# szaguldo-kamaz/FRI-ReinforcementLearning-C

Measured on AMD Instinct MI355X. Metric: rule-distance evals/sec (rules x envs), higher is better.
Workload: dtype f64; 1 GPU; cfg4_acrobot_64k_x_8k_per_gpu; nant=5, universe_len=41, rules_per_env=65536, envs_per_gpu=8192, exact_hits=4, dist_backend=none, world_size=1

## Files before the change

fri-reinforcementlearning-c_amd/csrc/five_rule_distance.hip:

```cpp
#include <stdlib.h>

#include <type_traits>

#include "device_common.h"

namespace frirl {

__device__ __forceinline__ void item_to_env_chunk(unsigned item, int cpe, int E, bool env_fastest, int &e, int &c)
{
    if (env_fastest) { c = (int)(item / (unsigned)E); e = (int)(item - (unsigned)c * (unsigned)E); }
    else { e = (int)(item / (unsigned)cpe); c = (int)(item - (unsigned)e * (unsigned)cpe); }
}

template <int NANT, bool WRITE, int UNROLL, int NT>
__global__ __launch_bounds__(FRIRL_BLOCK) void rule_distance_kernel(
    const double *__restrict__ u, const double *__restrict__ ve, int U, const double *__restrict__ rb,
    const int32_t *__restrict__ nrules, int maxR, const double *__restrict__ x, double *__restrict__ dists,
    uint32_t *__restrict__ hit, int rules_per_block, int cpe, int E, int env_fastest)
{
    int e, c;
    item_to_env_chunk(blockIdx.x, cpe, E, env_fastest != 0, e, c);
    const int R = nrules[e];
    const int r0 = c * rules_per_block;
    if (r0 >= R) return;
// ... 33 lines not shown
            if (rr < r_end) {
                double d0 = q[0] - v[j][0].x, d1 = q[0] - v[j][0].y;
                double a0 = d0 * d0, a1 = d1 * d1;
#pragma unroll
                for (int k = 1; k < NANT; k++) {
                    d0 = q[k] - v[j][k].x;
                    d1 = q[k] - v[j][k].y;
                    const double s0 = d0 * d0, s1 = d1 * d1;
                    a0 = a0 + s0;
                    a1 = a1 + s1;
                }
                double2 d;
                d.x = __dsqrt_rn(a0);
                d.y = __dsqrt_rn(a1);
                if (WRITE) {
                    if (NT == 1 || NT == 3) { __builtin_nontemporal_store(d.x, out + rr); __builtin_nontemporal_store(d.y, out + rr + 1); }
                    else *reinterpret_cast<double2 *>(out + rr) = d;
                }
                if (d.y == 0.0 && rr + 1 < R) best = min(best, (unsigned)(rr + 1));
                if (d.x == 0.0) best = min(best, (unsigned)rr);
            }
        }
    }
    best = block_min_u32(best, red_s);
    if (threadIdx.x == 0 && best != FRIRL_HIP_NO_HIT) atomicMin(&hit[e], best);
}

template <int NANT>
__device__ __forceinline__ double2 idx_pair_distance(const uint32_t (&w)[NANT], const double (&q)[NANT], const double *__restrict__ tab_s, int U)
{
    double2 t = lds_table_pair(tab_s, w[0]);
    double d0 = q[0] - t.x, d1 = q[0] - t.y;
    double a0 = d0 * d0, a1 = d1 * d1;
#pragma unroll
    for (int k = 1; k < NANT; k++) {
        t = lds_table_pair(tab_s + k * U, w[k]);
        d0 = q[k] - t.x;
        d1 = q[k] - t.y;
        const double s0 = d0 * d0, s1 = d1 * d1;
        a0 = a0 + s0;
        a1 = a1 + s1;
    }
    double2 d;
    d.x = __dsqrt_rn(a0);
    d.y = __dsqrt_rn(a1);
    return d;
}

template <int NANT, bool WRITE, int UNROLL, int BLOCK = FRIRL_BLOCK>
__global__ __launch_bounds__(BLOCK) void rule_distance_idx_kernel(
    const double *__restrict__ u, const double *__restrict__ ve, int U, const uint16_t *__restrict__ uidx,
    const int32_t *__restrict__ nrules, int maxR, const double *__restrict__ x, double *__restrict__ dists,
    uint32_t *__restrict__ hit, int rules_per_block, int cpe, int E, int env_fastest)
{
    extern __shared__ double tab_s[];
    int e, c;
    item_to_env_chunk(blockIdx.x, cpe, E, env_fastest != 0, e, c);
    const int R = nrules[e];
    const int r0 = c * rules_per_block;
    if (r0 >= R) return;
    int r_end = r0 + rules_per_block;
    if (r_end > R) r_end = R;

    __shared__ double q_s[NANT];
    __shared__ unsigned red_s[BLOCK / FRIRL_WAVE];
    for (int i = threadIdx.x; i < NANT * U; i += BLOCK) tab_s[i] = ve[i];
    if (threadIdx.x < NANT) q_s[threadIdx.x] = observe_ve(u, ve, U, threadIdx.x, x[(size_t)e * NANT + threadIdx.x]);
    __syncthreads();
    double q[NANT];
#pragma unroll
    for (int k = 0; k < NANT; k++) q[k] = q_s[k];

    const uint16_t *__restrict__ base = uidx + (size_t)e * NANT * maxR;
    double *__restrict__ out = WRITE ? dists + (size_t)e * maxR : nullptr;
    unsigned best = FRIRL_HIP_NO_HIT;
    constexpr int STEP = BLOCK * 2;

    for (int r = r0 + 2 * (int)threadIdx.x; r < r_end; r += STEP * UNROLL) {
        uint32_t w[UNROLL][NANT];
#pragma unroll
        for (int j = 0; j < UNROLL; j++) {
            const int rr = r + j * STEP;
            if (rr < r_end) {
#pragma unroll
                for (int k = 0; k < NANT; k++) w[j][k] = __builtin_nontemporal_load(reinterpret_cast<const uint32_t *>(base + (size_t)k * maxR + rr));
            }
        }
#pragma unroll
        for (int j = 0; j < UNROLL; j++) {
            const int rr = r + j * STEP;
            if (rr < r_end) {
                const double2 d = idx_pair_distance<NANT>(w[j], q, tab_s, U);
                if (WRITE) { __builtin_nontemporal_store(d.x, out + rr); __builtin_nontemporal_store(d.y, out + rr + 1); }
                if (d.y == 0.0 && rr + 1 < R) best = min(best, (unsigned)(rr + 1));
                if (d.x == 0.0) best = min(best, (unsigned)rr);
            }
        }
    }
    best = wave_min_u32(best);
    if ((threadIdx.x & (FRIRL_WAVE - 1)) == 0) red_s[threadIdx.x / FRIRL_WAVE] = best;
    __syncthreads();
    if (threadIdx.x == 0) {
        unsigned m = red_s[0];
        for (int w = 1; w < BLOCK / FRIRL_WAVE; w++) m = red_s[w] < m ? red_s[w] : m;
        if (m != FRIRL_HIP_NO_HIT) atomicMin(&hit[e], m);
    }
}

typedef uint32_t u32x2_t __attribute__((ext_vector_type(2)));
static constexpr int RD_XCDS = 8;

template <int BITS>
__device__ __forceinline__ double pk_table_entry(const double *__restrict__ tab_k, uint32_t w, int sh)
{
    constexpr uint32_t FM = ((1u << BITS) - 1u) << 3;
    const uint32_t off = (sh >= 3 ? (w >> (sh - 3)) : (w << (3 - sh))) & FM;
    return *reinterpret_cast<const double *>(reinterpret_cast<const char *>(tab_k) + off);
}

template <int NANT, int BITS>
__device__ __forceinline__ double2 pk_pair_distance(const u32x2_t (&w)[Packed<BITS>::words(NANT)], const double (&q)[NANT],
                                                    const double *__restrict__ tab_s)
{
    constexpr int FPW = Packed<BITS>::FPW, TS = 1 << BITS;
    double d0 = q[0] - pk_table_entry<BITS>(tab_s, w[0].x, 0), d1 = q[0] - pk_table_entry<BITS>(tab_s, w[0].y, 0);
    double a0 = d0 * d0, a1 = d1 * d1;
#pragma unroll
    for (int k = 1; k < NANT; k++) {
        const int sh = BITS * (k % FPW);
        d0 = q[k] - pk_table_entry<BITS>(tab_s + k * TS, w[k / FPW].x, sh);
        d1 = q[k] - pk_table_entry<BITS>(tab_s + k * TS, w[k / FPW].y, sh);
        const double s0 = d0 * d0, s1 = d1 * d1;
        a0 = a0 + s0;
        a1 = a1 + s1;
    }
    double2 d;
    d.x = __dsqrt_rn(a0);
    d.y = __dsqrt_rn(a1);
    return d;
}

__device__ __forceinline__ double sqrt_unscaled(double x)
{
    const double y = __builtin_amdgcn_rsq(x);
    const double s0 = x * y;
    const double h0 = y * 0.5;
    const double r0 = __builtin_fma(-h0, s0, 0.5);
    const double h1 = __builtin_fma(h0, r0, h0);
    const double s1 = __builtin_fma(s0, r0, s0);
    const double d0 = __builtin_fma(-s1, s1, x);
    const double s2 = __builtin_fma(d0, h1, s1);
    const double d1 = __builtin_fma(-s2, s2, x);
    const double r = __builtin_fma(d1, h1, s2);
    return x == 0.0 ? x : r;
}

__device__ __forceinline__ bool sq_in_unscaled_range(double s)
{
    return s == 0.0 || (s >= 0x1p-767 && s <= 0x1p1000);
}

template <int NANT, int BITS, bool FAST>
__device__ __forceinline__ void pk_pair_sq(const u32x2_t (&w)[Packed<BITS>::words(NANT)], const double *__restrict__ sq_s, double2 &d,
                                           bool &z0, bool &z1)
{
    constexpr int FPW = Packed<BITS>::FPW, TS = 1 << BITS;
    double a0 = pk_table_entry<BITS>(sq_s, w[0].x, 0), a1 = pk_table_entry<BITS>(sq_s, w[0].y, 0);
#pragma unroll
    for (int k = 1; k < NANT; k++) {
        const int sh = BITS * (k % FPW);
        a0 = a0 + pk_table_entry<BITS>(sq_s + k * TS, w[k / FPW].x, sh);
        a1 = a1 + pk_table_entry<BITS>(sq_s + k * TS, w[k / FPW].y, sh);
    }
    if (FAST) {
        d.x = sqrt_unscaled(a0);
        d.y = sqrt_unscaled(a1);
        z0 = a0 == 0.0;
        z1 = a1 == 0.0;
    } else {
        d.x = __dsqrt_rn(a0);
        d.y = __dsqrt_rn(a1);
        z0 = d.x == 0.0;
        z1 = d.y == 0.0;
    }
}

template <int NANT, int BITS, int BLOCK>
__device__ __forceinline__ bool fill_sq_table(const double *q_s, double *sq_s, const double (&tv)[(NANT * (1 << BITS) + BLOCK - 1) / BLOCK], int tid)
{
    constexpr int TS = 1 << BITS, N = NANT * TS;
    bool ok = true;
#pragma unroll
    for (int m = 0; m < (N + BLOCK - 1) / BLOCK; m++) {
        const int i = tid + m * BLOCK;
        if (N % BLOCK == 0 || i < N) {
            const double d = q_s[i >> BITS] - tv[m];
            const double s = d * d;
            sq_s[i] = s;
            ok = ok && sq_in_unscaled_range(s);
        }
    }
    return ok;
}

template <int NANT, int BITS, int BLOCK>
__device__ __forceinline__ void load_sq_sources(const double *__restrict__ ve, int U, double (&tv)[(NANT * (1 << BITS) + BLOCK - 1) / BLOCK], int tid)
{
    constexpr int TS = 1 << BITS, N = NANT * TS;
#pragma unroll
    for (int m = 0; m < (N + BLOCK - 1) / BLOCK; m++) {
        const int i = tid + m * BLOCK;
        const int k = i >> BITS, j = i & (TS - 1);
        tv[m] = (i < N && j < U) ? ve[k * U + j] : 0.0;
    }
}

template <int NANT, int BITS, bool DIGIT = false>
__global__ __launch_bounds__(FRIRL_BLOCK) void sq_tables_kernel(const double *__restrict__ u, const double *__restrict__ ve, int U, int E,
                                                              const double *__restrict__ x, double *__restrict__ sqtab,
                                                              uint32_t *__restrict__ fastv, uint32_t *__restrict__ hit,
                                                              const uint8_t *__restrict__ dict = nullptr)
{
    constexpr int TS = 1 << BITS, N = NANT * TS;
    __shared__ double q_s[FRIRL_WAVES_PER_BLOCK][NANT];
    const int lane = threadIdx.x & (FRIRL_WAVE - 1), wave = threadIdx.x / FRIRL_WAVE;
    const int e = blockIdx.x * FRIRL_WAVES_PER_BLOCK + wave;
    const bool live = e < E;
    double tv[(N + FRIRL_WAVE - 1) / FRIRL_WAVE];
    if constexpr (DIGIT) {
#pragma unroll
        for (int m = 0; m < (N + FRIRL_WAVE - 1) / FRIRL_WAVE; m++) {
            const int i = lane + m * FRIRL_WAVE;
            const int k = i >> BITS;
            const int idx = i < N ? (int)dict[i] : U;
            tv[m] = idx < U ? ve[k * U + idx] : 0.0;
        }
    } else {
        load_sq_sources<NANT, BITS, FRIRL_WAVE>(ve, U, tv, lane);
    }
    if (live && lane < NANT) q_s[wave][lane] = observe_ve(u, ve, U, lane, x[(size_t)e * NANT + lane]);
    __syncthreads();
    if (!live) return;
    const bool ok = fill_sq_table<NANT, BITS, FRIRL_WAVE>(q_s[wave], sqtab + (size_t)e * N, tv, lane);
    const bool fast = __all(ok);
    if (lane == 0) {
        fastv[e] = fast ? 1u : 0u;
        hit[e] = FRIRL_HIP_NO_HIT;
    }
}

template <int NANT, bool WRITE, int UNROLL, int BITS, bool SQ, bool PRE = false>
__global__ __launch_bounds__(FRIRL_BLOCK) void rule_distance_pk_kernel(
    const double *__restrict__ u, const double *__restrict__ ve, int U, const uint32_t *__restrict__ pidx,
    const int32_t *__restrict__ nrules, int maxR, const double *__restrict__ x, const double *__restrict__ qv, double *__restrict__ dists,
    uint32_t *__restrict__ hit, int rules_per_block, int cpe, int E, int env_fastest, const double *__restrict__ sqtab = nullptr,
    const uint32_t *__restrict__ fastv = nullptr)
{
    static_assert(SQ || !PRE, "the pre-pass serves the squared-difference form");
    constexpr int W = Packed<BITS>::words(NANT), TS = 1 << BITS;
    __shared__ __attribute__((aligned(16))) double tab_s[NANT * TS];
    __shared__ double q_s[NANT];
    __shared__ unsigned red_s[FRIRL_WAVES_PER_BLOCK];
    int e, c;
    if (PRE && env_fastest == 0) {
        const unsigned grp = blockIdx.x / (unsigned)(RD_XCDS * cpe), j = blockIdx.x - grp * (unsigned)(RD_XCDS * cpe);
        e = (int)(grp * RD_XCDS + j % RD_XCDS);
        c = (int)(j / RD_XCDS);
        if (e >= E) return;
    } else {
        item_to_env_chunk(blockIdx.x, cpe, E, env_fastest == 1, e, c);
    }
    const int R = nrules[e];
    const int r0 = c * rules_per_block;
    if (r0 >= R) return;
    int r_end = r0 + rules_per_block;
    if (r_end > R) r_end = R;

    const uint32_t *__restrict__ base = pidx + (size_t)e * W * maxR;
    constexpr int STEP = FRIRL_BLOCK * 2;
    u32x2_t w[UNROLL][W];
    auto load = [&](int r) {
#pragma unroll
        for (int j = 0; j < UNROLL; j++) {
            const int rr = r + j * STEP;
            if (rr < r_end) {
#pragma unroll
                for (int k = 0; k < W; k++) w[j][k] = __builtin_nontemporal_load(reinterpret_cast<const u32x2_t *>(base + (size_t)k * maxR + rr));
            }
        }
    };
    int r = r0 + 2 * (int)threadIdx.x;
    load(r);
    double *__restrict__ out = WRITE ? dists + (size_t)e * maxR : nullptr;
    unsigned best = FRIRL_HIP_NO_HIT;

    if constexpr (SQ) {
        double *sq_s = tab_s;
        bool fast;
        if constexpr (PRE) {
            constexpr int N2 = NANT * TS / 2;
            const double2 *__restrict__ src = reinterpret_cast<const double2 *>(sqtab + (size_t)e * (NANT * TS));
            for (int i = threadIdx.x; i < N2; i += FRIRL_BLOCK) reinterpret_cast<double2 *>(sq_s)[i] = src[i];
            fast = fastv[e] != 0u;
            __syncthreads();
        } else {
            double tv[(NANT * TS + FRIRL_BLOCK - 1) / FRIRL_BLOCK];
            load_sq_sources<NANT, BITS, FRIRL_BLOCK>(ve, U, tv, (int)threadIdx.x);
// ... 356 lines not shown
static void launch_pk_form(const frirl_hip_tables *t, const frirl_hip_rulebases *b, const uint32_t *pidx, const double *x, const double *qv,
                           double *ruledists, uint32_t *hit, hipStream_t s, const RdGrid &g, bool sq)
{
    if (sq) launch_pk<NANT, UN, true>(t, b, pidx, x, qv, ruledists, hit, s, g);
    else launch_pk<NANT, UN, false>(t, b, pidx, x, nullptr, ruledists, hit, s, g);
}

template <int NANT, int UN>
static void launch_pk_pre(const frirl_hip_tables *t, const frirl_hip_rulebases *b, const uint32_t *pidx, const double *x, double *ruledists,
                          uint32_t *hit, void *ws, hipStream_t s, const RdGrid &g)
{
    double *sqtab = static_cast<double *>(ws);
    uint32_t *fastv = reinterpret_cast<uint32_t *>(sqtab + (size_t)b->E * NANT * (1 << RD_PK_BITS));
    const int order = frirl_host::opts().rd_order;
    const unsigned items = order == 0 ? (unsigned)g.cpe * (unsigned)((b->E + RD_XCDS - 1) / RD_XCDS * RD_XCDS) : g.items;
    hipLaunchKernelGGL((sq_tables_kernel<NANT, RD_PK_BITS>), dim3((unsigned)((b->E + FRIRL_WAVES_PER_BLOCK - 1) / FRIRL_WAVES_PER_BLOCK)), dim3(FRIRL_BLOCK),
                       0, s, t->u, t->ve, t->U, b->E, x, sqtab, fastv, hit);
    if (ruledists)
        hipLaunchKernelGGL((rule_distance_pk_kernel<NANT, true, UN, RD_PK_BITS, true, true>), dim3(items), dim3(FRIRL_BLOCK), 0, s, t->u, t->ve, t->U, pidx,
                           b->nrules, b->maxR, x, nullptr, ruledists, hit, g.rules_per_block, g.cpe, b->E, order, sqtab, fastv);
    else
        hipLaunchKernelGGL((rule_distance_pk_kernel<NANT, false, UN, RD_PK_BITS, true, true>), dim3(items), dim3(FRIRL_BLOCK), 0, s, t->u, t->ve, t->U, pidx,
                           b->nrules, b->maxR, x, nullptr, ruledists, hit, g.rules_per_block, g.cpe, b->E, order, sqtab, fastv);
}

template <int NANT>
static int launch_packed(const frirl_hip_tables *t, const frirl_hip_rulebases *b, const uint32_t *pidx, const double *x,
                         double *ruledists, uint32_t *hit, void *ws, hipStream_t s)
{
    using namespace frirl_host;
    const RdTune tn = rd_tune();
    const bool sq = opts().rd_sqdiff != 0;
    const bool pre = ws && sq && opts().rd_prepass != 0;
    const int UP = pre ? RdPkConfig<NANT>::UNROLL_PRE : RdPkConfig<NANT>::UNROLL;
    const int un = (NANT <= 5 && tn.unroll) ? tn.unroll : UP;
    const bool qpass = sq && !pre && opts().rd_qpass == 1;
    RdGrid g;
    if (!make_grid(b, tn.chunk > 0 ? tn.chunk : 2 * FRIRL_BLOCK * un, g)) { set_error("five_hip_rule_distance_packed: too many work items"); return FRIRL_HIP_EINVAL; }
    if (pre) {
        if ((long)g.cpe * ((long)b->E + RD_XCDS) > 0x7FFFFFFFL) { set_error("five_hip_rule_distance_packed_ws: too many work items"); return FRIRL_HIP_EINVAL; }
        if constexpr (NANT <= 5) {
            if (un == 8) launch_pk_pre<NANT, 8>(t, b, pidx, x, ruledists, hit, ws, s, g);
            else if (un == 2) launch_pk_pre<NANT, 2>(t, b, pidx, x, ruledists, hit, ws, s, g);
            else if (un == 1) launch_pk_pre<NANT, 1>(t, b, pidx, x, ruledists, hit, ws, s, g);
            else launch_pk_pre<NANT, 4>(t, b, pidx, x, ruledists, hit, ws, s, g);
        } else {
            launch_pk_pre<NANT, RdPkConfig<NANT>::UNROLL_PRE>(t, b, pidx, x, ruledists, hit, ws, s, g);
        }
        return check_launch("five_hip_rule_distance_packed_ws");
    }
    void *scratch = nullptr;
    const double *qv = nullptr;
    if (qpass) {
        const size_t qv_off = 256, bytes = qv_off + sizeof(double) * (size_t)b->E * NANT;
        const hipError_t e1 = hipMallocAsync(&scratch, bytes, s);
        if (e1 != hipSuccess) { (void)hipGetLastError(); set_error("five_hip_rule_distance_packed: hipMallocAsync(%zu B) failed: %s", bytes, hipGetErrorString(e1)); return FRIRL_HIP_ELAUNCH; }
        double *q = reinterpret_cast<double *>(static_cast<char *>(scratch) + qv_off);
        const int nq = b->E * NANT;
        hipLaunchKernelGGL(observe_reset_kernel, dim3((nq + 255) / 256), dim3(256), 0, s, t->u, t->ve, t->U, NANT, b->E, x, q, hit, static_cast<unsigned *>(scratch));
        qv = q;
    } else if (hipMemsetAsync(hit, 0xFF, sizeof(uint32_t) * (size_t)b->E, s) != hipSuccess) {
        return check_launch("five_hip_rule_distance_packed(memset)");
    }
    if constexpr (NANT <= 5) {
        if (un == 4) launch_pk_form<NANT, 4>(t, b, pidx, x, qv, ruledists, hit, s, g, sq);
        else if (un == 2) launch_pk_form<NANT, 2>(t, b, pidx, x, qv, ruledists, hit, s, g, sq);
        else if (un == 1) launch_pk_form<NANT, 1>(t, b, pidx, x, qv, ruledists, hit, s, g, sq);
        else launch_pk_form<NANT, RdPkConfig<NANT>::UNROLL>(t, b, pidx, x, qv, ruledists, hit, s, g, sq);
    } else {
        launch_pk_form<NANT, RdPkConfig<NANT>::UNROLL>(t, b, pidx, x, qv, ruledists, hit, s, g, sq);
    }
    if (scratch && hipFreeAsync(scratch, s) != hipSuccess) { set_error("five_hip_rule_distance_packed: hipFreeAsync failed"); return FRIRL_HIP_ELAUNCH; }
    return check_launch("five_hip_rule_distance_packed");
}

static constexpr int RD_CD_TILE = 2 * FRIRL_BLOCK * 4;
static constexpr int RD_CD_TILE_BYTES = 3 * RD_CD_TILE;
static constexpr int RD_CD_MAX_NANT = 5, RD_CD_FIELDS = (RD_CD_MAX_NANT + 1) / 2;

struct CodeParams {
    uint32_t shift[RD_CD_FIELDS], mask[RD_CD_FIELDS], da[RD_CD_FIELDS], magic[RD_CD_FIELDS];
};

static int ceil_log2(uint32_t n)
{
    int b = 0;
    while ((1u << b) < n) b++;
    return b;
}

static bool code_params(int nant, const int32_t *d, CodeParams &cp)
{
    if (nant < 1 || nant > RD_CD_MAX_NANT || !d) return false;
    int total = 0;
    for (int f = 0; f < RD_CD_FIELDS; f++) cp.shift[f] = cp.mask[f] = 0u, cp.da[f] = 1u, cp.magic[f] = 1u << 18;
    for (int k = 0; k < nant; k += 2) {
        const int f = k / 2;
        if (d[k] < 1 || d[k] > 64 || (k + 1 < nant && (d[k + 1] < 1 || d[k + 1] > 64))) return false;
        const uint32_t da = (uint32_t)d[k], db = k + 1 < nant ? (uint32_t)d[k + 1] : 1u;
        const int bits = ceil_log2(da * db);
        if (bits > 12) return false;
        cp.shift[f] = (uint32_t)total;
        cp.mask[f] = (1u << bits) - 1u;
        cp.da[f] = da;
        cp.magic[f] = ((1u << 18) + da - 1u) / da;
        total += bits;
    }
    return total <= 24;
}

static size_t coded_bytes(int nant, int U, long E, long maxR, const int32_t *d)
{
    CodeParams cp;
    if (!packed_words(nant, U) || E < 1 || maxR < 2 || !code_params(nant, d, cp)) return 0;
    return (size_t)E * (size_t)((maxR + RD_CD_TILE - 1) / RD_CD_TILE) * RD_CD_TILE_BYTES;
}

__global__ __launch_bounds__(FRIRL_BLOCK) void pack_codes_kernel(const uint16_t *__restrict__ uidx, const int32_t *__restrict__ nrules, int nant, int maxR,
                                                                 int tpe, long ntiles, const uint8_t *__restrict__ rank, CodeParams cp,
                                                                 uint8_t *__restrict__ codes)
{
    const int t = threadIdx.x;
    for (long tile = blockIdx.x; tile < ntiles; tile += gridDim.x) {
        const long e = tile / tpe;
        const int c = (int)(tile - e * tpe);
        const int R = nrules[e];
        const int Rp = min(R + (R & 1), maxR);
        const uint16_t *__restrict__ src = uidx + (size_t)e * nant * maxR;
        uint32_t code[8];
#pragma unroll
        for (int i = 0; i < 8; i++) {
            const int r = c * RD_CD_TILE + 2 * t + (i & 1) + 2 * FRIRL_BLOCK * (i >> 1);
            uint32_t v = 0u;
            if (r < Rp) {
                for (int k = 0; k < nant; k += 2) {
                    const uint32_t ja = rank[k * 64 + (src[(size_t)k * maxR + r] & 63u)];
                    const uint32_t jb = k + 1 < nant ? rank[(k + 1) * 64 + (src[(size_t)(k + 1) * maxR + r] & 63u)] : 0u;
                    v |= (jb * cp.da[k / 2] + ja) << cp.shift[k / 2];
                }
            }
            code[i] = v & 0xFFFFFFu;
        }
        u32x2_t *__restrict__ dst = reinterpret_cast<u32x2_t *>(codes + (size_t)tile * RD_CD_TILE_BYTES + 8 * t);
        u32x2_t p0, p1, p2;
        p0.x = code[0] | code[1] << 24;  p0.y = code[1] >> 8 | code[2] << 16;
        p1.x = code[2] >> 16 | code[3] << 8;  p1.y = code[4] | code[5] << 24;
        p2.x = code[5] >> 8 | code[6] << 16;  p2.y = code[6] >> 16 | code[7] << 8;
        dst[0] = p0;
        dst[RD_CD_TILE / 8] = p1;
        dst[2 * (RD_CD_TILE / 8)] = p2;
    }
}

template <int NANT>
__device__ __forceinline__ double cd_rule_sq(uint32_t code, const double *__restrict__ sq_s, const CodeParams &cp)
{
    constexpr int TS = 64;
    double a = 0.0;
#pragma unroll
    for (int k = 0; k < NANT; k += 2) {
        const int f = k / 2;
        const uint32_t v = (code >> cp.shift[f]) & cp.mask[f];
        if (k + 1 < NANT) {
            const uint32_t jb = __umul24(v, cp.magic[f]) >> 18;
            const uint32_t ja = v - __umul24(jb, cp.da[f]);
            const double sa = *reinterpret_cast<const double *>(reinterpret_cast<const char *>(sq_s + k * TS) + (ja << 3));
            const double sb = *reinterpret_cast<const double *>(reinterpret_cast<const char *>(sq_s + (k + 1) * TS) + (jb << 3));
            a = k == 0 ? sa : a + sa;
            a = a + sb;
        } else {
            const double sa = *reinterpret_cast<const double *>(reinterpret_cast<const char *>(sq_s + k * TS) + (v << 3));
            a = k == 0 ? sa : a + sa;
        }
    }
    return a;
}

template <int NANT, bool WRITE>
__global__ __launch_bounds__(FRIRL_BLOCK) void rule_distance_cd_kernel(const uint8_t *__restrict__ codes, const int32_t *__restrict__ nrules, int maxR,
                                                                     double *__restrict__ dists, uint32_t *__restrict__ hit, int cpe, int E,
                                                                     const double *__restrict__ sqtab, const uint32_t *__restrict__ fastv, CodeParams cp)
{
    constexpr int TS = 64, STEP = FRIRL_BLOCK * 2;
    __shared__ __attribute__((aligned(16))) double sq_s[NANT * TS];
    __shared__ unsigned red_s[FRIRL_WAVES_PER_BLOCK];
    const unsigned grp = blockIdx.x / (unsigned)(RD_XCDS * cpe), gj = blockIdx.x - grp * (unsigned)(RD_XCDS * cpe);
    const int e = (int)(grp * RD_XCDS + gj % RD_XCDS);
    const int c = (int)(gj / RD_XCDS);
    if (e >= E) return;
    const int R = nrules[e];
    const int r0 = c * RD_CD_TILE;
    if (r0 >= R) return;
    int r_end = r0 + RD_CD_TILE;
    if (r_end > R) r_end = R;

    const int r = r0 + 2 * (int)threadIdx.x;
    const bool any = r < r_end;
    u32x2_t w[3];
    if (any) {
        const uint8_t *__restrict__ src = codes + ((size_t)e * cpe + c) * RD_CD_TILE_BYTES + 8 * threadIdx.x;
#pragma unroll
        for (int m = 0; m < 3; m++) w[m] = __builtin_nontemporal_load(reinterpret_cast<const u32x2_t *>(src + m * RD_CD_TILE));
    }
    constexpr int N2 = NANT * TS / 2;
    const double2 *__restrict__ tsrc = reinterpret_cast<const double2 *>(sqtab + (size_t)e * (NANT * TS));
    for (int i = threadIdx.x; i < N2; i += FRIRL_BLOCK) reinterpret_cast<double2 *>(sq_s)[i] = tsrc[i];
    const bool fast = fastv[e] != 0u;
    __syncthreads();

    double *__restrict__ out = WRITE ? dists + (size_t)e * maxR : nullptr;
    unsigned best = FRIRL_HIP_NO_HIT;
    auto sweep = [&](auto fast_tag) {
        constexpr bool FAST = decltype(fast_tag)::value;
        if (!any) return;
        uint32_t code[8];
        code[0] = w[0].x;
        code[1] = __builtin_amdgcn_alignbit(w[0].y, w[0].x, 24);
        code[2] = __builtin_amdgcn_alignbit(w[1].x, w[0].y, 16);
        code[3] = w[1].x >> 8;
        code[4] = w[1].y;
        code[5] = __builtin_amdgcn_alignbit(w[2].x, w[1].y, 24);
        code[6] = __builtin_amdgcn_alignbit(w[2].y, w[2].x, 16);
        code[7] = w[2].y >> 8;
#pragma unroll
        for (int j = 0; j < 4; j++) {
            const int rr = r + j * STEP;
            if (rr < r_end) {
                const double a0 = cd_rule_sq<NANT>(code[2 * j], sq_s, cp), a1 = cd_rule_sq<NANT>(code[2 * j + 1], sq_s, cp);
                double2 d;
                bool z0, z1;
                if (FAST) {
                    d.x = sqrt_unscaled(a0);
                    d.y = sqrt_unscaled(a1);
                    z0 = a0 == 0.0;
                    z1 = a1 == 0.0;
                } else {
                    d.x = __dsqrt_rn(a0);
                    d.y = __dsqrt_rn(a1);
                    z0 = d.x == 0.0;
                    z1 = d.y == 0.0;
                }
                if (WRITE) { __builtin_nontemporal_store(d.x, out + rr); __builtin_nontemporal_store(d.y, out + rr + 1); }
                if (z1 && rr + 1 < R) best = min(best, (unsigned)(rr + 1));
                if (z0) best = min(best, (unsigned)rr);
            }
        }
    };
    if (fast) sweep(std::true_type{});
    else sweep(std::false_type{});
    best = wave_min_u32(best);
    if ((threadIdx.x & (FRIRL_WAVE - 1)) == 0) red_s[threadIdx.x / FRIRL_WAVE] = best;
    __syncthreads();
    if (threadIdx.x == 0) {
        unsigned m = red_s[0];
        for (int v = 1; v < FRIRL_WAVES_PER_BLOCK; v++) m = red_s[v] < m ? red_s[v] : m;
        if (m != FRIRL_HIP_NO_HIT) atomicMin(&hit[e], m);
    }
}

template <int NANT>
static int launch_coded(const frirl_hip_tables *t, const frirl_hip_rulebases *b, const uint8_t *codes, const uint8_t *dict, const CodeParams &cp,
                        const double *x, double *ruledists, uint32_t *hit, void *ws, hipStream_t s)
{
    using namespace frirl_host;
    const long cpe = ((long)b->maxR + RD_CD_TILE - 1) / RD_CD_TILE;
    if (cpe * ((long)b->E + RD_XCDS) > 0x7FFFFFFFL) { set_error("five_hip_rule_distance_coded_ws: too many work items"); return FRIRL_HIP_EINVAL; }
    double *sqtab = static_cast<double *>(ws);
    uint32_t *fastv = reinterpret_cast<uint32_t *>(sqtab + (size_t)b->E * NANT * (1 << RD_PK_BITS));
    const unsigned items = (unsigned)cpe * (unsigned)((b->E + RD_XCDS - 1) / RD_XCDS * RD_XCDS);
    hipLaunchKernelGGL((sq_tables_kernel<NANT, RD_PK_BITS, true>), dim3((unsigned)((b->E + FRIRL_WAVES_PER_BLOCK - 1) / FRIRL_WAVES_PER_BLOCK)), dim3(FRIRL_BLOCK),
                       0, s, t->u, t->ve, t->U, b->E, x, sqtab, fastv, hit, dict);
    if (ruledists)
        hipLaunchKernelGGL((rule_distance_cd_kernel<NANT, true>), dim3(items), dim3(FRIRL_BLOCK), 0, s, codes, b->nrules, b->maxR, ruledists, hit, (int)cpe,
                           b->E, sqtab, fastv, cp);
    else
        hipLaunchKernelGGL((rule_distance_cd_kernel<NANT, false>), dim3(items), dim3(FRIRL_BLOCK), 0, s, codes, b->nrules, b->maxR, ruledists, hit, (int)cpe,
                           b->E, sqtab, fastv, cp);
    return check_launch("five_hip_rule_distance_coded_ws");
}

__global__ void sqrt_unscaled_check_kernel(const double *__restrict__ a, double *__restrict__ fast, double *__restrict__ ref, long n)
{
    const long i = (long)blockIdx.x * blockDim.x + threadIdx.x;
    if (i >= n) return;
    fast[i] = sqrt_unscaled(a[i]);
    ref[i] = __dsqrt_rn(a[i]);
}

template <int NANT>
__global__ __launch_bounds__(FRIRL_BLOCK) void sq_guard_kernel(const double *__restrict__ u, const double *__restrict__ ve, int U,
                                                             const double *__restrict__ x, int32_t *__restrict__ ok)
{
    constexpr int TS = 1 << RD_PK_BITS;
    __shared__ double sq_s[NANT * TS];
    __shared__ double q_s[NANT];
    const int e = blockIdx.x;
    double tv[(NANT * TS + FRIRL_BLOCK - 1) / FRIRL_BLOCK];
    load_sq_sources<NANT, RD_PK_BITS, FRIRL_BLOCK>(ve, U, tv, (int)threadIdx.x);
    if (threadIdx.x < NANT) q_s[threadIdx.x] = observe_ve(u, ve, U, threadIdx.x, x[(size_t)e * NANT + threadIdx.x]);
    __syncthreads();
    const bool fast = !__syncthreads_or(!fill_sq_table<NANT, RD_PK_BITS, FRIRL_BLOCK>(q_s, sq_s, tv, (int)threadIdx.x));
    if (threadIdx.x == 0) ok[e] = fast ? 1 : 0;
}

}

extern "C" int five_hip_rule_distance_uses_uidx(int32_t nant, int32_t U)
{
    return nant >= 1 && nant <= FRIRL_HIP_MAX_NANT && U <= 65536 && sizeof(double) * nant * (size_t)U <= 150 * 1024 && !frirl_host::opts().no_uidx;
}

extern "C" int five_hip_rule_distance(const frirl_hip_tables *t, const frirl_hip_rulebases *b, const double *x,
                                      double *ruledists, uint32_t *hit, void *stream)
{
    using namespace frirl_host;
    int rc = check_rulebases(t, b);
    if (rc) return rc;
    if (!x || !hit) { set_error("five_hip_rule_distance: NULL x/hit"); return FRIRL_HIP_EINVAL; }
    if (ruledists && (reinterpret_cast<uintptr_t>(ruledists) & 15)) { set_error("five_hip_rule_distance: ruledists must be 16-byte aligned"); return FRIRL_HIP_EINVAL; }
    if ((rc = check_device())) return rc;
    hipStream_t s = as_stream(stream);

    switch (t->nant) {
#define FRIRL_CASE(N) case N: return frirl::launch_nant<N>(t, b, x, ruledists, hit, s);
        FRIRL_CASE(1) FRIRL_CASE(2) FRIRL_CASE(3) FRIRL_CASE(4) FRIRL_CASE(5) FRIRL_CASE(6) FRIRL_CASE(7) FRIRL_CASE(8)
        FRIRL_CASE(9) FRIRL_CASE(10) FRIRL_CASE(11) FRIRL_CASE(12) FRIRL_CASE(13) FRIRL_CASE(14) FRIRL_CASE(15) FRIRL_CASE(16)
#undef FRIRL_CASE
    }
    set_error("five_hip_rule_distance: unsupported nant=%d", t->nant);
    return FRIRL_HIP_EINVAL;
}

extern "C" int five_hip_rule_distance_packed_words(int32_t nant, int32_t U)
{
    return frirl::packed_words(nant, U);
}

extern "C" int frirl_hip_pack_indices(const frirl_hip_tables *t, const frirl_hip_rulebases *b, uint32_t *pidx, void *stream)
{
    using namespace frirl_host;
    int rc = check_rulebases(t, b);
    if (rc) return rc;
    if (!b->uidx || !pidx) { set_error("frirl_hip_pack_indices: NULL uidx/pidx"); return FRIRL_HIP_EINVAL; }
    if (!frirl::packed_words(t->nant, t->U)) { set_error("frirl_hip_pack_indices: nant=%d U=%d is not served by the packed form", t->nant, t->U); return FRIRL_HIP_EINVAL; }
    if ((rc = check_device())) return rc;
    const long total = (long)b->E * b->maxR;
    long grid = (total + FRIRL_BLOCK - 1) / FRIRL_BLOCK;
    if (grid > (long)frirl::device_cus() * 32) grid = (long)frirl::device_cus() * 32;
    hipLaunchKernelGGL(frirl::pack_indices_kernel<frirl::RD_PK_BITS>, dim3((unsigned)grid), dim3(FRIRL_BLOCK), 0, as_stream(stream), b->uidx, t->nant,
                       b->maxR, total, pidx);
    return check_launch("frirl_hip_pack_indices");
}

extern "C" int five_hip_sqrt_unscaled_check(const double *a, double *fast, double *ref, int64_t n, void *stream)
{
    using namespace frirl_host;
    if (n < 0 || (n && (!a || !fast || !ref))) { set_error("five_hip_sqrt_unscaled_check: bad arguments"); return FRIRL_HIP_EINVAL; }
    int rc = check_device();
    if (rc) return rc;
    if (n) hipLaunchKernelGGL(frirl::sqrt_unscaled_check_kernel, dim3((unsigned)((n + 255) / 256)), dim3(256), 0, as_stream(stream), a, fast, ref, (long)n);
    return check_launch("five_hip_sqrt_unscaled_check");
}

extern "C" int five_hip_rule_distance_sq_guard(const frirl_hip_tables *t, int32_t E, const double *x, int32_t *ok, void *stream)
{
    using namespace frirl_host;
    int rc = check_tables(t);
    if (rc) return rc;
    if (!frirl::packed_words(t->nant, t->U)) { set_error("five_hip_rule_distance_sq_guard: nant=%d U=%d is not served by the packed form", t->nant, t->U); return FRIRL_HIP_EINVAL; }
    if (E < 0 || (E && (!x || !ok))) { set_error("five_hip_rule_distance_sq_guard: bad arguments"); return FRIRL_HIP_EINVAL; }
    if ((rc = check_device())) return rc;
    if (!E) return 0;
    switch (t->nant) {
#define FRIRL_CASE(N) case N: hipLaunchKernelGGL(frirl::sq_guard_kernel<N>, dim3((unsigned)E), dim3(FRIRL_BLOCK), 0, as_stream(stream), t->u, t->ve, t->U, x, ok); break;
        FRIRL_CASE(1) FRIRL_CASE(2) FRIRL_CASE(3) FRIRL_CASE(4) FRIRL_CASE(5) FRIRL_CASE(6) FRIRL_CASE(7) FRIRL_CASE(8)
        FRIRL_CASE(9) FRIRL_CASE(10) FRIRL_CASE(11) FRIRL_CASE(12) FRIRL_CASE(13) FRIRL_CASE(14) FRIRL_CASE(15) FRIRL_CASE(16)
#undef FRIRL_CASE
    }
    return check_launch("five_hip_rule_distance_sq_guard");
}

static int rule_distance_packed(const frirl_hip_tables *t, const frirl_hip_rulebases *b, const uint32_t *pidx, const double *x,
                                double *ruledists, uint32_t *hit, void *ws, void *stream)
{
    using namespace frirl_host;
    int rc;
    const Options &o = opts();
    if (!frirl::packed_words(t->nant, t->U) || !o.rd_packed || o.no_uidx || o.rd_persist == 1)
        return five_hip_rule_distance(t, b, x, ruledists, hit, stream);
    if (!pidx || !x || !hit) { set_error("five_hip_rule_distance_packed: NULL pidx/x/hit"); return FRIRL_HIP_EINVAL; }
    if (reinterpret_cast<uintptr_t>(pidx) & 7) { set_error("five_hip_rule_distance_packed: pidx must be 8-byte aligned"); return FRIRL_HIP_EINVAL; }
    if (ruledists && (reinterpret_cast<uintptr_t>(ruledists) & 15)) { set_error("five_hip_rule_distance_packed: ruledists must be 16-byte aligned"); return FRIRL_HIP_EINVAL; }
    if ((rc = check_device())) return rc;
    hipStream_t s = as_stream(stream);

    switch (t->nant) {
#define FRIRL_CASE(N) case N: return frirl::launch_packed<N>(t, b, pidx, x, ruledists, hit, ws, s);
        FRIRL_CASE(1) FRIRL_CASE(2) FRIRL_CASE(3) FRIRL_CASE(4) FRIRL_CASE(5) FRIRL_CASE(6) FRIRL_CASE(7) FRIRL_CASE(8)
        FRIRL_CASE(9) FRIRL_CASE(10) FRIRL_CASE(11) FRIRL_CASE(12) FRIRL_CASE(13) FRIRL_CASE(14) FRIRL_CASE(15) FRIRL_CASE(16)
#undef FRIRL_CASE
    }
    set_error("five_hip_rule_distance_packed: unsupported nant=%d", t->nant);
    return FRIRL_HIP_EINVAL;
}

extern "C" int five_hip_rule_distance_packed(const frirl_hip_tables *t, const frirl_hip_rulebases *b, const uint32_t *pidx, const double *x,
                                             double *ruledists, uint32_t *hit, void *stream)
{
    const int rc = frirl_host::check_rulebases(t, b);
    return rc ? rc : rule_distance_packed(t, b, pidx, x, ruledists, hit, nullptr, stream);
}

extern "C" size_t five_hip_rule_distance_packed_workspace_bytes(int32_t nant, int32_t U, int32_t E)
{
    return frirl::packed_ws_bytes(nant, U, E);
}

extern "C" int five_hip_rule_distance_packed_ws(const frirl_hip_tables *t, const frirl_hip_rulebases *b, const uint32_t *pidx, const double *x,
                                                double *ruledists, uint32_t *hit, void *workspace, size_t workspace_bytes, void *stream)
{
    using namespace frirl_host;
    const int rc = check_rulebases(t, b);
    if (rc) return rc;
    const size_t need = frirl::packed_ws_bytes(t->nant, t->U, b->E);
    if (need) {
        if (!workspace || workspace_bytes < need) {
            set_error("five_hip_rule_distance_packed_ws: workspace of %zu B at %p, nant=%d U=%d E=%d needs %zu B "
                      "(five_hip_rule_distance_packed_workspace_bytes)", workspace_bytes, workspace, t->nant, t->U, b->E, need);
            return FRIRL_HIP_EINVAL;
        }
// ... 67 lines not shown
```

Baseline: 524.4 billion evals/s.

## Pre-scale rule codes, defer exact-hit search to rare second pass, drop block reduction

Rule codes are pre-shifted by 3 so decoded fields serve directly as byte offsets into the shared squared-distance tables, and the decode uses a negated multiplier with mul24 in place of a subtract. The per-rule zero check is replaced by a running minimum of the high word of each squared sum. The exact first-hit search runs only when some lane saw a zero, recomputing those rules in a second pass and using per-wave atomics instead of the shared-memory block reduction and its barrier. It also swaps the group division for a host-computed multiply-high and makes the fast sqrt clamp with fmax rather than special-casing zero, trading a rare recompute for less per-rule work in the common path.

```diff
diff --git a/fri-reinforcementlearning-c_amd/csrc/five_rule_distance.hip b/fri-reinforcementlearning-c_amd/csrc/five_rule_distance.hip
--- a/fri-reinforcementlearning-c_amd/csrc/five_rule_distance.hip
+++ b/fri-reinforcementlearning-c_amd/csrc/five_rule_distance.hip
@@ -209,7 +209,7 @@
     const double s2 = __builtin_fma(d0, h1, s1);
     const double d1 = __builtin_fma(-s2, s2, x);
     const double r = __builtin_fma(d1, h1, s2);
-    return x == 0.0 ? x : r;
+    return __builtin_fmax(r, 0.0);
 }
 
 __device__ __forceinline__ bool sq_in_unscaled_range(double s)
@@ -872,39 +872,65 @@
     }
 }
 
+static constexpr uint32_t RD_CD_Q8 = 127u << 3;
+struct CodeScan {
+    uint32_t shift[RD_CD_FIELDS], mask8[RD_CD_FIELDS], magic[RD_CD_FIELDS];
+    int32_t negda[RD_CD_FIELDS];
+    __device__ __forceinline__ explicit CodeScan(const CodeParams &cp)
+    {
+#pragma unroll
+        for (int f = 0; f < RD_CD_FIELDS; f++) shift[f] = cp.shift[f], mask8[f] = (cp.mask[f] & 0xFFFu) << 3, magic[f] = cp.magic[f], negda[f] = -(int32_t)cp.da[f];
+    }
+};
+
+__device__ __forceinline__ double cd_table_entry(const double *__restrict__ tab_k, uint32_t off8)
+{
+    return *reinterpret_cast<const double *>(reinterpret_cast<const char *>(tab_k) + off8);
+}
+
 template <int NANT>
-__device__ __forceinline__ double cd_rule_sq(uint32_t code, const double *__restrict__ sq_s, const CodeParams &cp)
+__device__ __forceinline__ double cd_rule_sq(uint32_t code8, const double *__restrict__ sq_s, const CodeScan &cs)
 {
     constexpr int TS = 64;
     double a = 0.0;
 #pragma unroll
     for (int k = 0; k < NANT; k += 2) {
         const int f = k / 2;
-        const uint32_t v = (code >> cp.shift[f]) & cp.mask[f];
+        const uint32_t v8 = (f == 0 ? code8 : code8 >> cs.shift[f]) & cs.mask8[f];
         if (k + 1 < NANT) {
-            const uint32_t jb = __umul24(v, cp.magic[f]) >> 18;
-            const uint32_t ja = v - __umul24(jb, cp.da[f]);
-            const double sa = *reinterpret_cast<const double *>(reinterpret_cast<const char *>(sq_s + k * TS) + (ja << 3));
-            const double sb = *reinterpret_cast<const double *>(reinterpret_cast<const char *>(sq_s + (k + 1) * TS) + (jb << 3));
+            const uint32_t jb8 = (__umul24(v8, cs.magic[f]) >> 18) & RD_CD_Q8;
+            const uint32_t ja8 = (uint32_t)(__mul24((int)jb8, cs.negda[f]) + (int)v8);
+            const double sa = cd_table_entry(sq_s + k * TS, ja8);
+            const double sb = cd_table_entry(sq_s + (k + 1) * TS, jb8);
             a = k == 0 ? sa : a + sa;
             a = a + sb;
         } else {
-            const double sa = *reinterpret_cast<const double *>(reinterpret_cast<const char *>(sq_s + k * TS) + (v << 3));
+            const double sa = cd_table_entry(sq_s + k * TS, v8);
             a = k == 0 ? sa : a + sa;
         }
     }
     return a;
+}
+
+struct GroupDiv { uint32_t mul, shift; };
+static GroupDiv group_div(uint32_t d)
+{
+    const int l = ceil_log2(d);
+    GroupDiv g;
+    g.mul = (uint32_t)(((1ull << (31 + l)) + d - 1) / d);
+    g.shift = (uint32_t)(l - 1);
+    return g;
 }
 
 template <int NANT, bool WRITE>
 __global__ __launch_bounds__(FRIRL_BLOCK) void rule_distance_cd_kernel(const uint8_t *__restrict__ codes, const int32_t *__restrict__ nrules, int maxR,
                                                                      double *__restrict__ dists, uint32_t *__restrict__ hit, int cpe, int E,
-                                                                     const double *__restrict__ sqtab, const uint32_t *__restrict__ fastv, CodeParams cp)
+                                                                     const double *__restrict__ sqtab, const uint32_t *__restrict__ fastv, CodeParams cp,
+                                                                     GroupDiv gd)
 {
     constexpr int TS = 64, STEP = FRIRL_BLOCK * 2;
     __shared__ __attribute__((aligned(16))) double sq_s[NANT * TS];
-    __shared__ unsigned red_s[FRIRL_WAVES_PER_BLOCK];
-    const unsigned grp = blockIdx.x / (unsigned)(RD_XCDS * cpe), gj = blockIdx.x - grp * (unsigned)(RD_XCDS * cpe);
+    const unsigned grp = __umulhi(blockIdx.x, gd.mul) >> gd.shift, gj = blockIdx.x - grp * (unsigned)(RD_XCDS * cpe);
     const int e = (int)(grp * RD_XCDS + gj % RD_XCDS);
     const int c = (int)(gj / RD_XCDS);
     if (e >= E) return;
@@ -926,56 +952,65 @@
     const double2 *__restrict__ tsrc = reinterpret_cast<const double2 *>(sqtab + (size_t)e * (NANT * TS));
     for (int i = threadIdx.x; i < N2; i += FRIRL_BLOCK) reinterpret_cast<double2 *>(sq_s)[i] = tsrc[i];
     const bool fast = fastv[e] != 0u;
+    const CodeScan cs(cp);
     __syncthreads();
 
     double *__restrict__ out = WRITE ? dists + (size_t)e * maxR : nullptr;
-    unsigned best = FRIRL_HIP_NO_HIT;
+    uint32_t code[8];
+    uint32_t lo = ~0u;
     auto sweep = [&](auto fast_tag) {
         constexpr bool FAST = decltype(fast_tag)::value;
-        if (!any) return;
-        uint32_t code[8];
-        code[0] = w[0].x;
-        code[1] = __builtin_amdgcn_alignbit(w[0].y, w[0].x, 24);
-        code[2] = __builtin_amdgcn_alignbit(w[1].x, w[0].y, 16);
-        code[3] = w[1].x >> 8;
-        code[4] = w[1].y;
-        code[5] = __builtin_amdgcn_alignbit(w[2].x, w[1].y, 24);
-        code[6] = __builtin_amdgcn_alignbit(w[2].y, w[2].x, 16);
-        code[7] = w[2].y >> 8;
 #pragma unroll
         for (int j = 0; j < 4; j++) {
             const int rr = r + j * STEP;
             if (rr < r_end) {
-                const double a0 = cd_rule_sq<NANT>(code[2 * j], sq_s, cp), a1 = cd_rule_sq<NANT>(code[2 * j + 1], sq_s, cp);
+                const double a0 = cd_rule_sq<NANT>(code[2 * j], sq_s, cs), a1 = cd_rule_sq<NANT>(code[2 * j + 1], sq_s, cs);
                 double2 d;
-                bool z0, z1;
                 if (FAST) {
                     d.x = sqrt_unscaled(a0);
                     d.y = sqrt_unscaled(a1);
-                    z0 = a0 == 0.0;
-                    z1 = a1 == 0.0;
+                    lo = min(lo, min((uint32_t)__double2hiint(a0), (uint32_t)__double2hiint(a1)));
                 } else {
                     d.x = __dsqrt_rn(a0);
                     d.y = __dsqrt_rn(a1);
-                    z0 = d.x == 0.0;
-                    z1 = d.y == 0.0;
+                    lo = min(lo, min((uint32_t)__double2hiint(d.x), (uint32_t)__double2hiint(d.y)));
                 }
                 if (WRITE) { __builtin_nontemporal_store(d.x, out + rr); __builtin_nontemporal_store(d.y, out + rr + 1); }
+            }
+        }
+    };
+    auto first_hit = [&](auto fast_tag) -> unsigned {
+        constexpr bool FAST = decltype(fast_tag)::value;
+        unsigned best = FRIRL_HIP_NO_HIT;
+#pragma unroll
+        for (int j = 0; j < 4; j++) {
+            const int rr = r + j * STEP;
+            if (rr < r_end) {
+                const double a0 = cd_rule_sq<NANT>(code[2 * j], sq_s, cs), a1 = cd_rule_sq<NANT>(code[2 * j + 1], sq_s, cs);
+                const bool z0 = FAST ? a0 == 0.0 : __dsqrt_rn(a0) == 0.0, z1 = FAST ? a1 == 0.0 : __dsqrt_rn(a1) == 0.0;
                 if (z1 && rr + 1 < R) best = min(best, (unsigned)(rr + 1));
                 if (z0) best = min(best, (unsigned)rr);
             }
         }
+        return best;
     };
-    if (fast) sweep(std::true_type{});
-    else sweep(std::false_type{});
+    if (any) {
+        code[0] = w[0].x << 3;
+        code[1] = __builtin_amdgcn_alignbit(w[0].y, w[0].x, 21);
+        code[2] = __builtin_amdgcn_alignbit(w[1].x, w[0].y, 13);
+        code[3] = w[1].x >> 5;
+        code[4] = w[1].y << 3;
+        code[5] = __builtin_amdgcn_alignbit(w[2].x, w[1].y, 21);
+        code[6] = __builtin_amdgcn_alignbit(w[2].y, w[2].x, 13);
+        code[7] = w[2].y >> 5;
+        if (fast) sweep(std::true_type{});
+        else sweep(std::false_type{});
+    }
+    if (!__any(lo == 0u)) return;
+    unsigned best = FRIRL_HIP_NO_HIT;
+    if (any) best = fast ? first_hit(std::true_type{}) : first_hit(std::false_type{});
     best = wave_min_u32(best);
-    if ((threadIdx.x & (FRIRL_WAVE - 1)) == 0) red_s[threadIdx.x / FRIRL_WAVE] = best;
-    __syncthreads();
-    if (threadIdx.x == 0) {
-        unsigned m = red_s[0];
-        for (int v = 1; v < FRIRL_WAVES_PER_BLOCK; v++) m = red_s[v] < m ? red_s[v] : m;
-        if (m != FRIRL_HIP_NO_HIT) atomicMin(&hit[e], m);
-    }
+    if ((threadIdx.x & (FRIRL_WAVE - 1)) == 0 && best != FRIRL_HIP_NO_HIT) atomicMin(&hit[e], best);
 }
 
 template <int NANT>
@@ -988,14 +1023,15 @@
     double *sqtab = static_cast<double *>(ws);
     uint32_t *fastv = reinterpret_cast<uint32_t *>(sqtab + (size_t)b->E * NANT * (1 << RD_PK_BITS));
     const unsigned items = (unsigned)cpe * (unsigned)((b->E + RD_XCDS - 1) / RD_XCDS * RD_XCDS);
+    const GroupDiv gd = group_div((uint32_t)(RD_XCDS * cpe));
     hipLaunchKernelGGL((sq_tables_kernel<NANT, RD_PK_BITS, true>), dim3((unsigned)((b->E + FRIRL_WAVES_PER_BLOCK - 1) / FRIRL_WAVES_PER_BLOCK)), dim3(FRIRL_BLOCK),
                        0, s, t->u, t->ve, t->U, b->E, x, sqtab, fastv, hit, dict);
     if (ruledists)
         hipLaunchKernelGGL((rule_distance_cd_kernel<NANT, true>), dim3(items), dim3(FRIRL_BLOCK), 0, s, codes, b->nrules, b->maxR, ruledists, hit, (int)cpe,
-                           b->E, sqtab, fastv, cp);
+                           b->E, sqtab, fastv, cp, gd);
     else
         hipLaunchKernelGGL((rule_distance_cd_kernel<NANT, false>), dim3(items), dim3(FRIRL_BLOCK), 0, s, codes, b->nrules, b->maxR, ruledists, hit, (int)cpe,
-                           b->E, sqtab, fastv, cp);
+                           b->E, sqtab, fastv, cp, gd);
     return check_launch("five_hip_rule_distance_coded_ws");
 }
 
```

New measurement: 546.8 billion evals/s (median of 6 runs). 4.3% higher.
